# IvanIZ/BenchPush

Measured on AMD Instinct MI355X. Metric: env-steps/sec at N=4096 envs (ship-ice-v0), 1/2/4/8 MI355X, higher is better.
Workload: dtype f64

## Files before the change

benchpush_amd/csrc/bp_device.hpp:

```cpp
#pragma once
#include <hip/hip_runtime.h>
#include <stdint.h>

#include "../../include/benchpush_amd.h"

#define BP_KADJ 24
#define BP_ACAP 64

typedef double2 d2;

enum { BODY_DYNAMIC = 0, BODY_KINEMATIC = 1, BODY_STATIC = 2 };
__device__ __forceinline__ int kind_ctype(int k) { return k & 0xFF; }
__device__ __forceinline__ int kind_group(int k) { return (k >> 8) & 0xFF; }
__device__ __forceinline__ int kind_btype(int k) { return (k >> 16) & 3; }
enum { ARB_FIRST = 0, ARB_NORMAL = 1, ARB_IGNORE = 2, ARB_CACHED = 3 };
#define ARB_FREE_KEY 0xFFFFFFFFu

struct DevParams {
    double dt_sub;
    int steps, iterations, persistence, settle_steps;
    double damping_pow, bias_coef, slop, target_speed, max_yaw_rate, map_w, map_h, goal_y, m_to_pix;
    double beta, boundary_penalty, terminal_reward, local_w, local_h, vshift, obs_range;
    double goal_x, goal_reach, k_increment;
    int env_kind;
// ... 101 lines not shown
__device__ __forceinline__ double fclampd(double f, double lo, double hi) { return fmin(fmax(f, lo), hi); }

#define HW_PLANE_A(h) ((int)((h) & 31ull))
#define HW_PLANE_B(h) ((int)(((h) >> 5) & 31ull))
#define HW_VERT_A(h) ((int)(((h) >> 10) & 31ull))
#define HW_VERT_B(h) ((int)(((h) >> 15) & 31ull))
#define HW_NV_A(h) ((int)(((h) >> 20) & 31ull))
#define HW_NV_B(h) ((int)(((h) >> 25) & 31ull))
#define HW_HAS_A (1ull << 32)
#define HW_HAS_B (1ull << 33)
#define HW_PRIM_B (1ull << 34)
#define HW_BOTH (1ull << 35)
#define BP_SUPPORT_MARGIN 1e-10
#define BP_TIE_TOL 1e-9
#ifndef BP_QCAP
#define BP_QCAP 96
#endif

#define BP_CC_IDX_BITS 14
#define BP_EVCAP 32
#define BP_MBOX 16
#ifndef BP_NSLOT
#define BP_NSLOT 96
#endif
#define BP_PROFN 64
#define BP_SNAP_ROWS 9
#define BP_SNAP_COLS 12

struct LdsMap {
    unsigned sv, sw, sb, sp, ag, tf, q_dir, q_c, r_val, q_meta, q_aux, r_idx, pt_a, pt_thr, cc, cc_hw, res_smA, res_smB, res_iA, res_iB, res_jA, res_jB, mvs, owner, colmask, mvo, sbody, mv,
        slot_of, rf, ev_d, ev_key, ctl, snap, prof, total;
};
__host__ __device__ inline LdsMap bp_lds_map(const int nbcap, const int mvcap, const bool box, const bool prof)
{
    LdsMap m;
    unsigned p = 0;
    m.sv = p; p += 16u * (BP_NSLOT + 1);
    m.sw = p; p += 16u * (BP_NSLOT + 1);
    m.sb = p; p += 16u * (BP_NSLOT + 1);
    m.sp = p; p += 16u * (BP_NSLOT + 1);
    m.ag = p; p += 32u;
    m.tf = p;
    m.q_dir = p; p += 16u * BP_QCAP;
    m.q_c = p; p += 8u * BP_QCAP;
    m.r_val = p; p += 8u * BP_QCAP;
    m.q_meta = p; p += 4u * BP_QCAP;
    m.q_aux = p; p += 4u * BP_QCAP;
    m.r_idx = p; p += 4u * BP_QCAP;
    m.pt_a = p; p += 16u * 64;
    m.pt_thr = p; p += 16u * 64;
    m.cc = p; p += 8u * 64;
    m.cc_hw = p; p += 8u * 64;
    m.res_smA = p; p += 8u * 64;
    m.res_smB = p; p += 8u * 64;
    m.res_iA = p; p += 4u * 64;
    m.res_iB = p; p += 4u * 64;
    m.res_jA = p; p += 4u * 64;
    m.res_jB = p; p += 4u * 64;
    m.mvs = p; p += 4u * (unsigned)nbcap;
    m.owner = p; p += 2u * (BP_NSLOT + 2);
    m.colmask = p; p += 2u * (BP_NSLOT + 2);
    m.mvo = p; p += 4u * (BP_NSLOT + 2);
    m.sbody = p; p += 2u * (BP_NSLOT + 2);
    m.mv = p; p += 2u * (unsigned)mvcap;
    m.slot_of = p; p += (unsigned)nbcap;
    m.rf = p; p += 64u;
    p = (p + 15u) & ~15u;
    m.ev_d = p; if (box) p += 16u * 3 * BP_EVCAP;
    m.ev_key = p; if (box) p += 4u * BP_EVCAP;
    p = (p + 7u) & ~7u;
    m.ctl = p; if (box) p += 8u * 4;
    m.snap = p; if (box) p += 8u * BP_SNAP_ROWS * BP_SNAP_COLS;
    m.prof = p; if (prof) p += 8u * BP_PROFN;
    m.total = (p + 15u) & ~15u;
    return m;
}

struct BpImgHdr {
    unsigned stamp, stamp_start, costp, n_post, n_contact, n_first, ship_post, ship_contacts;
    int nmv, nslots, nlevels, yaw_violated, boundary_violated, wall_flag, cc_ok, cc_kmax, quiescent, pad_;
    unsigned long long prev_amask;
    double curr_dt, total_ke, total_imp, ecoef_e, ecoef;
};
#define BP_IMG_DROWS 20
#define BP_IMG_UROWS 11
#define BP_IMG_HDR 256
static_assert(sizeof(BpImgHdr) <= BP_IMG_HDR, "park image header");
__host__ __device__ inline unsigned bp_img_regs_off(const unsigned lds_bytes) { return (lds_bytes + 1023u) & ~1023u; }
__host__ __device__ inline unsigned bp_img_bytes(const unsigned lds_bytes) { return bp_img_regs_off(lds_bytes) + 512u * BP_IMG_DROWS + 256u * BP_IMG_UROWS + BP_IMG_HDR; }

#define SQ_MAXLEV 32
#define BP_DBL_MIN 2.2250738585072014e-308
#define BP_PI 3.14159265358979323846
#define BP_INF (__builtin_inf())

__device__ __forceinline__ void bp_sincos(double x, double &sn, double &cs)
{
    const double invpio2 = 6.36619772367581382433e-01;
    const double pio2_1 = 1.57079632673412561417e+00, pio2_1t = 6.07710050650619224932e-11;
    const double pio2_2 = 6.07710050630396597660e-11, pio2_2t = 2.02226624879595063154e-21;
    const double S1 = -1.66666666666666324348e-01, S2 = 8.33333333332248946124e-03, S3 = -1.98412698298579493134e-04,
                 S4 = 2.75573137070700676789e-06, S5 = -2.50507602534068634195e-08, S6 = 1.58969099521155010221e-10;
    const double C1 = 4.16666666666666019037e-02, C2 = -1.38888888888741095749e-03, C3 = 2.48015872894767294178e-05,
                 C4 = -2.75573143513906633035e-07, C5 = 2.08757232129817482790e-09, C6 = -1.13596475577881948265e-11;
    double fn = __builtin_rint(x * invpio2);
    double r = x - fn * pio2_1;
    double w = fn * pio2_1t;
    double y0 = r - w;
    const bool deep = __builtin_fabs(y0) < __builtin_fabs(x) * 7.62939453125e-06;
// ... 109 lines not shown
```

benchpush_amd/csrc/bp_physics.hpp:

```cpp
#pragma once
#include "bp_device.hpp"
#include <type_traits>

#ifdef BP_PROF
#define PROF_DECL unsigned long long _pt = __builtin_amdgcn_s_memtime();
#define PROF_ACC(slot) { unsigned long long _n = __builtin_amdgcn_s_memtime(); if (lane_id() == 0) L.prof[slot] += _n - _pt; _pt = _n; }
#define PROF_CNT(slot, v) { const unsigned long long _v = (unsigned long long)(v); if (lane_id() == 0) L.prof[slot] += _v; }
#define PROF_MAX(slot, v) { const unsigned long long _v = (unsigned long long)(v); if (lane_id() == 0 && _v > L.prof[slot]) L.prof[slot] = _v; }
#else
#define PROF_DECL
#define PROF_ACC(slot)
#define PROF_CNT(slot, v)
#define PROF_MAX(slot, v)
#endif


#define BP_UNLIKELY(x) __builtin_expect(!!(x), 0)
#define BP_UNLIKELY2(x) __builtin_expect(!!(x), 0)
#ifdef BP_DEBUG_PATHS
#define BP_DBGP(bit) ((P.dbg_paths & (bit)) != 0)
#define BP_TRACE_ON(D) ((D).dbg != nullptr)
#else
#define BP_DBGP(bit) false
#define BP_TRACE_ON(D) false
#endif
#ifndef BP_BOUND_GROUPS
#define BP_BOUND_GROUPS 3
#endif
#include "bp_contact.hpp"

struct EnvCtx {
    int nb;
    const int *nv;
    const d2 *lv, *ln;
    const double4 *mass;
    const double4 *prop;
    const int *kind;
    d2 *pxy, *rot, *wv, *wn, *pv;
    double *ang;
    double4 *bb, *fat;
    unsigned short *adj;
    unsigned char *adjn;
    unsigned long long *hint;
};

template <typename T> __device__ __forceinline__ T &gE(T *const base, const int idx) { return *(T *)((char *)base + (size_t)((unsigned)idx * (unsigned)sizeof(T))); }

struct LdsCtx {
    d2 *sv, *sw, *sb;
    d2 *ag;
    d2 *sp;
    unsigned char *slot_of;
    unsigned *mvs;
    unsigned short *owner;
    unsigned short *colmask;
    d2 *tf;
    unsigned short *mv;
    unsigned *mvo;
    unsigned short *sbody;
    unsigned char *rf;
    unsigned long long *res_smA, *res_smB;
    unsigned *res_iA, *res_iB, *res_jA, *res_jB;
    d2 *q_dir;
    double *q_c, *r_val;
    unsigned *q_meta, *q_aux, *r_idx;
    uint4 *pt_a;
    d2 *pt_thr;
    unsigned long long *cc, *cc_hw;
    d2 *mbox;
    unsigned *ev_key;
    d2 *ev_d;
    double *ctl;
    unsigned long long *snap;
#ifdef BP_PROF
    unsigned long long *prof;
#endif
};

struct SubState {
    unsigned stamp;
// ... 92 lines not shown
}

__device__ __forceinline__ void world_from_pose(const DevParams &P, const EnvCtx &E, int i, bool active, int q, double4 t,
                                                double4 &outbb)
{
    const int n = active ? gE(E.nv, i) : 0;
    const bool valid = active && (q < n);
    double vx = 0, vy = 0;
    if (valid) {
        const d2 lv = gE(E.lv, i * BP_MAXV + q), ln = gE(E.ln, i * BP_MAXV + q);
        const double c = t.x, s = t.y;
        vx = (c * lv.x + (-s) * lv.y) + t.z;
        vy = (s * lv.x + c * lv.y) + t.w;
        const double nx = c * ln.x + (-s) * ln.y;
        const double ny = s * ln.x + c * ln.y;
        gE(E.wv, i * BP_MAXV + q) = mk2(vx, vy);
        gE(E.wn, i * BP_MAXV + q) = mk2(nx, ny);
    }
    const double l = half_min(valid ? vx : BP_INF);
    const double r = half_max(valid ? vx : -BP_INF);
    const double bo = half_min(valid ? vy : BP_INF);
    const double tp = half_max(valid ? vy : -BP_INF);
    const double rad = gE(E.prop, i).x;
    outbb.x = l - rad; outbb.y = bo - rad; outbb.z = r + rad; outbb.w = tp + rad;
}

template <int VL>
__device__ __forceinline__ void support_queries(const EnvCtx &E, const LdsCtx &L, const int nq)
{
    const int lane = lane_id();
    const int l8 = lane & 7, g = lane >> 3;
    for (int base = 0; base < nq; base += 8) {
        const int k = base + g;
        const bool act = k < nq;
        const d2 dir = L.q_dir[act ? k : 0];
        const unsigned meta = L.q_meta[act ? k : 0];
        const int body = (int)(meta & 0xFFFFu), nv = (int)(meta >> 16);
        double best = BP_INF;
        int bi = 255;
#pragma unroll
        for (int t = 0; t < (VL + 7) / 8; t++) {
            const int q = l8 + 8 * t;
            const bool ok = act && (q < nv);
            const d2 v = gE(E.wv, body * BP_MAXV + (ok ? q : 0));
            const double d = vdot(dir, v);
            if (ok && d < best) { best = d; bi = q; }
        }
        const double m = oct_min_f64(best);
        const int mi = oct_min_i32((best == m) ? bi : 255);
        if (act && best == m && bi == mi) { L.r_val[k] = best; L.r_idx[k] = (unsigned)bi; }
    }
}

template <int KIND, bool DAMP = false>
__device__ __forceinline__ void substep(const DevParams &P, const EnvCtx &E, const LdsCtx &L, ArbReg &A, SubState &S,
                                        const double dt, const int ship_rules)
{
    const int lane = lane_id();
    constexpr int VL = (KIND == BP_ENV_BOX) ? 4 : (KIND == BP_ENV_MAZE) ? 8 : BP_MAXV;
    if (KIND == BP_ENV_BOX) { S.nev = 0; S.evmask = 0ull; }
    S.stamp += 1u;
    const unsigned now = S.stamp;
    const double prev_dt = S.curr_dt;
    S.curr_dt = dt;
    if (A.key != ARB_FREE_KEY && A.stamp == now - 1u) A.state = ARB_NORMAL;
    PROF_DECL
    PROF_CNT(16, S.nmv)

    for (int k0 = 0; k0 < S.nmv; k0 += 64) {
        const int k = k0 + lane;
        double rad = 0.0;
        double4 fatb; fatb.x = fatb.y = -BP_INF; fatb.z = fatb.w = BP_INF;
        if (k < S.nmv) {
            const int i = L.mv[k];
            const int sl = L.slot_of[i];
            d2 v = mk2(0.0, 0.0), w2 = mk2(0.0, 0.0), vb = mk2(0.0, 0.0);
            if (sl != 255) { v = L.sv[sl]; w2 = L.sw[sl]; vb = L.sb[sl]; }
            d2 p = gE(E.pxy, i);
            if (sl != 255) p = L.sp[sl];
            const double a = gE(E.ang, i);
            d2 r = gE(E.rot, i);
            const double4 ms = gE(E.mass, i);
            rad = gE(E.prop, i).x;
            fatb = gE(E.fat, i);
            L.rf[lane] = (unsigned char)gE(E.nv, i);
            p.x = p.x + (v.x + vb.x) * dt;
            p.y = p.y + (v.y + vb.y) * dt;
            const double a2 = a + (w2.x + w2.y) * dt;
            if (a2 != a) { double sn, cs; bp_sincos(a2, sn, cs); r = mk2(cs, sn); }
            gE(E.pxy, i) = p; gE(E.ang, i) = a2; gE(E.rot, i) = r;
            if (i == 0) { L.ag[0] = mk2(a2, 0.0); L.ag[1] = r; }
            if (sl != 255) { L.sb[sl] = mk2(0.0, 0.0); L.sw[sl].y = 0.0; L.sp[sl] = p; }
            double4 t;
            t.x = r.x; t.y = r.y;
            t.z = p.x - (ms.z * r.x - ms.w * r.y);
            t.w = p.y - (ms.z * r.y + ms.w * r.x);
            L.tf[2 * lane] = mk2(t.x, t.y);
            L.tf[2 * lane + 1] = mk2(t.z, t.w);
            L.mvs[i] = now;
        }
        const int cnt = min(64, S.nmv - k0);
        unsigned long long *bbk = L.res_smA;
        if (lane < cnt) { bbk[lane * 4 + 0] = ~0ull; bbk[lane * 4 + 1] = 0ull; bbk[lane * 4 + 2] = ~0ull; bbk[lane * 4 + 3] = 0ull; }
        lds_sync();
        PROF_ACC(33)
        for (int t0 = 0; t0 < cnt * VL; t0 += 64) {
            const int t = t0 + lane;
            const int kk = t / VL, q = t - kk * VL;
            if (kk < cnt) {
                const int i = L.mv[k0 + kk];
                if (q < (int)L.rf[kk]) {
                    const d2 t0_ = L.tf[2 * kk], t1_ = L.tf[2 * kk + 1];
// ... 122 lines not shown
        {
            const double dm = vdot(fnA, vAm), d0 = vdot(fnA, vA0), dp = vdot(fnA, vAp);
            if (evA && cnB == nB_h && cnB >= 2 && d0 + BP_SUPPORT_MARGIN <= dm && d0 + BP_SUPPORT_MARGIN <= dp && !BP_DBGP(4)) { sepAc = (d0 - cA) + 0.0; qryA = false; }
        }
        {
            const double dm = vdot(fnB, vBm), d0 = vdot(fnB, vB0), dp = vdot(fnB, vBp);
            if (evB && cnA == nA_h && cnA >= 2 && d0 + BP_SUPPORT_MARGIN <= dm && d0 + BP_SUPPORT_MARGIN <= dp && !BP_DBGP(4)) { sepBc = (d0 - cB) + 0.0; qryB = false; }
        }
        {
            const unsigned long long mqA = ballot(qryA), mqB = ballot(qryB);
            const int nqA = __popcll(mqA), nq1 = nqA + __popcll(mqB);
            PROF_CNT(37, nq1)
            if (BP_UNLIKELY(nq1)) {
                const int slA = popc_below(mqA, lane), slB = nqA + popc_below(mqB, lane);
                for (int q0 = 0; q0 < nq1; q0 += BP_QCAP) {
                    const bool inA = qryA && slA >= q0 && slA < q0 + BP_QCAP, inB = qryB && slB >= q0 && slB < q0 + BP_QCAP;
                    if (inA) { L.q_dir[slA - q0] = fnA; L.q_meta[slA - q0] = (unsigned)sb | ((unsigned)nB_h << 16); }
                    if (inB) { L.q_dir[slB - q0] = fnB; L.q_meta[slB - q0] = (unsigned)sa | ((unsigned)nA_h << 16); }
                    lds_sync();
                    support_queries<VL>(E, L, min(nq1 - q0, BP_QCAP));
                    lds_sync();
                    if (inA) { sepAc = (L.r_val[slA - q0] - cA) + 0.0; jAc = (int)L.r_idx[slA - q0]; }
                    if (inB) { sepBc = (L.r_val[slB - q0] - cB) + 0.0; jBc = (int)L.r_idx[slB - q0]; }
                    lds_sync();
                }
            }
        }
        if (valid && (sepAc > rsum || sepBc > rsum)) {
            valid = false;
            if (hw & HW_BOTH) {
                const unsigned long long nh = (hw & ~(HW_BOTH | HW_PRIM_B)) | ((sepAc > rsum) ? 0ull : HW_PRIM_B);
                gE(E.hint, i * BP_KADJ + s) = nh;
                if (base == 0) L.cc_hw[lane] = nh;
            }
        }
        const unsigned long long cm = ballot(valid);
        PROF_ACC(28)
        PROF_CNT(18, __popcll(cm))
        if (cm == 0) continue;
        PROF_CNT(25, 1)
        const int nc = __popcll(cm);
        const int myr = popc_below(cm, lane);
        const int nA_l = valid ? nA_h : 0, nB_l = valid ? nB_h : 0;
        if (valid) {
            uint4 pa;
            pa.x = (unsigned)sa | ((unsigned)sb << 16);
            pa.y = (unsigned)nA_l | (evA ? 0x80u : 0u) | ((unsigned)nB_l << 8) | ((unsigned)hA << 16) | ((unsigned)jAc << 24);
            pa.z = (unsigned)sb | ((unsigned)sa << 16);
            pa.w = (unsigned)nB_l | (evB ? 0x80u : 0u) | ((unsigned)nA_l << 8) | ((unsigned)hB << 16) | ((unsigned)jBc << 24);
            L.pt_a[myr] = pa;
            L.pt_thr[myr] = mk2(sepAc, sepBc);
            L.res_smA[myr] = evA ? f64_key(sepAc) : 0ull; L.res_iA[myr] = evA ? ((unsigned)hA << 8) | (unsigned)jAc : 0xFFFFFFFFu;
            L.res_smB[myr] = evB ? f64_key(sepBc) : 0ull; L.res_iB[myr] = evB ? ((unsigned)hB << 8) | (unsigned)jBc : 0xFFFFFFFFu;
        }
        lds_sync();
        {
            int nq = 0, g0 = 0;
            const uint2 *const pts = (const uint2 *)L.pt_a;
            const double *const pts_thr = (const double *)L.pt_thr;
            auto round_addr = [&](const uint2 e, int &pbody, int &qbody, int &np, int &nqv, int &hX, bool &evX, int &jc, int &jm, int &jp) {
                pbody = (int)(e.x & 0xFFFFu); qbody = (int)(e.x >> 16);
                np = (int)(e.y & 0x7Fu); evX = (e.y & 0x80u) != 0; nqv = (int)((e.y >> 8) & 0xFFu);
                hX = (int)((e.y >> 16) & 0xFFu); jc = (int)(e.y >> 24);
                jm = (jc == 0) ? max(nqv, 1) - 1 : jc - 1; jp = (jc + 1 >= nqv) ? 0 : jc + 1;
            };
            int rr_start = nc;
            {
                constexpr int GW = (BP_BOUND_GROUPS == 3 && KIND != BP_ENV_BOX) ? BP_MAXV + 1 : 32, IPR = 64 / GW;
                static_assert(GW >= BP_MAXV && IPR * GW <= 64, "a lane group holds every plane of a side");
                const int g = lane / GW, f = lane - g * GW;
                const int ipr = BP_DBGP(16) ? 1 : IPR;
                bool fits = !BP_DBGP(2);
                for (int r0 = 0; r0 < nc && fits; r0 += ipr) {
                    const bool on0 = g < ipr && 2 * r0 + g < 2 * nc, on1 = g < ipr && 2 * r0 + ipr + g < 2 * nc;
                    const int ta = on0 ? 2 * r0 + g : 2 * r0, tb = on1 ? 2 * r0 + ipr + g : 2 * r0;
                    const uint2 e0 = pts[ta], e1 = pts[tb];
                    const double th0 = pts_thr[ta], th1 = pts_thr[tb];
                    int pb0, qb0, np0, nqv0, hX0, jc0, jm0, jp0, pb1, qb1, np1, nqv1, hX1, jc1, jm1, jp1; bool ev0, ev1;
                    round_addr(e0, pb0, qb0, np0, nqv0, hX0, ev0, jc0, jm0, jp0);
                    round_addr(e1, pb1, qb1, np1, nqv1, hX1, ev1, jc1, jm1, jp1);
                    const int fc0 = (f < np0) ? f : 0, fc1 = (f < np1) ? f : 0;
                    const d2 fn0 = gE(E.wn, pb0 * BP_MAXV + fc0), fp0 = gE(E.wv, pb0 * BP_MAXV + fc0), vb0 = gE(E.wv, qb0 * BP_MAXV + jc0), vm0 = gE(E.wv, qb0 * BP_MAXV + jm0), vp0 = gE(E.wv, qb0 * BP_MAXV + jp0);
                    const d2 fn1 = gE(E.wn, pb1 * BP_MAXV + fc1), fp1 = gE(E.wv, pb1 * BP_MAXV + fc1), vb1 = gE(E.wv, qb1 * BP_MAXV + jc1), vm1 = gE(E.wv, qb1 * BP_MAXV + jm1), vp1 = gE(E.wv, qb1 * BP_MAXV + jp1);
                    {
                        const bool pv = on0 && (f < np0) && !(ev0 && f == hX0);
                        const double c = vdot(fn0, fp0);
                        const double bound = (fmin(vdot(fn0, vb0), fmin(vdot(fn0, vm0), vdot(fn0, vp0))) - c) + 0.0;
                        const bool surv = pv && (!ev0 || bound >= th0);
                        const unsigned long long sm = ballot(surv);
                        const int sl = nq + popc_below(sm, lane);
                        if (surv && sl < BP_QCAP) {
                            L.q_dir[sl] = fn0; L.q_meta[sl] = (unsigned)qb0 | ((unsigned)nqv0 << 16);
                            L.q_aux[sl] = (unsigned)(ta >> 1) | ((unsigned)(ta & 1) << 8) | ((unsigned)f << 16);
                            L.q_c[sl] = c;
                        }
                        nq += __popcll(sm);
                    }
                    {
                        const bool pv = on1 && (f < np1) && !(ev1 && f == hX1);
                        const double c = vdot(fn1, fp1);
                        const double bound = (fmin(vdot(fn1, vb1), fmin(vdot(fn1, vm1), vdot(fn1, vp1))) - c) + 0.0;
                        const bool surv = pv && (!ev1 || bound >= th1);
                        const unsigned long long sm = ballot(surv);
                        const int sl = nq + popc_below(sm, lane);
                        if (surv && sl < BP_QCAP) {
                            L.q_dir[sl] = fn1; L.q_meta[sl] = (unsigned)qb1 | ((unsigned)nqv1 << 16);
// ... 20 lines not shown
                        const int sl = s0 + lane;
                        if (sl < nq) {
                            const unsigned aux = L.q_aux[sl];
                            const int r = (int)(aux & 0xFFu);
                            const double sp = (L.r_val[sl] - L.q_c[sl]) + 0.0;
                            const unsigned long long key = f64_key(sp);
                            L.q_c[sl] = __builtin_bit_cast(double, key);
                            atomicMax((aux & 0x100u) ? &L.res_smB[r] : &L.res_smA[r], key);
                        }
                    }
                    lds_sync();
                    if (valid && myr >= g0 && myr < rr) {
                        if (evA && f64_key(sepAc) != L.res_smA[myr]) L.res_iA[myr] = 0xFFFFFFFFu;
                        if (evB && f64_key(sepBc) != L.res_smB[myr]) L.res_iB[myr] = 0xFFFFFFFFu;
                    }
                    lds_sync();
                    for (int s0 = 0; s0 < nq; s0 += 64) {
                        const int sl = s0 + lane;
                        if (sl < nq) {
                            const unsigned aux = L.q_aux[sl];
                            const int r = (int)(aux & 0xFFu);
                            const unsigned long long key = __builtin_bit_cast(unsigned long long, L.q_c[sl]);
                            if (key == ((aux & 0x100u) ? L.res_smB[r] : L.res_smA[r])) atomicMin((aux & 0x100u) ? &L.res_iB[r] : &L.res_iA[r], ((aux >> 16) << 8) | L.r_idx[sl]);
                        }
                    }
                    lds_sync();
                    nq = 0; g0 = rr;
                    PROF_ACC(30)
                }
                if (rr == nc) break;
                const uint2 e = pts[2 * rr + side];
                const double th = pts_thr[2 * rr + side];
                int pbody, qbody, np, nqv, hX, jc, jm, jp; bool evX;
                round_addr(e, pbody, qbody, np, nqv, hX, evX, jc, jm, jp);
                const bool pv = (f < np) && !(evX && f == hX);
                const int fc = (f < np) ? f : 0;
                const d2 fn = gE(E.wn, pbody * BP_MAXV + fc), fp = gE(E.wv, pbody * BP_MAXV + fc);
                const d2 vb = gE(E.wv, qbody * BP_MAXV + jc), vm = gE(E.wv, qbody * BP_MAXV + jm), vp = gE(E.wv, qbody * BP_MAXV + jp);
                const double c = vdot(fn, fp);
                const double bound = (fmin(vdot(fn, vb), fmin(vdot(fn, vm), vdot(fn, vp))) - c) + 0.0;
                const bool surv = pv && (!evX || bound >= th);
                const unsigned long long sm = ballot(surv);
                if (surv) {
                    const int sl = nq + popc_below(sm, lane);
                    L.q_dir[sl] = fn; L.q_meta[sl] = (unsigned)qbody | ((unsigned)nqv << 16);
                    L.q_aux[sl] = (unsigned)rr | ((unsigned)side << 8) | ((unsigned)f << 16);
                    L.q_c[sl] = c;
                }
                nq += __popcll(sm);
                lds_sync();
            }
        }
        PROF_ACC(3)
        Manifold M;
        M.count = 0; M.h0 = M.h1 = 0; M.n = mk2(0, 0);
        M.p1_0 = M.p2_0 = M.p1_1 = M.p2_1 = mk2(0, 0);
        bool touching = false;
        int src = 2;
        d2 n = mk2(0, 0);
        int iA = 0, iB = 0, jA = 0, jB = 0;
        int i1A = 0, i1B = 0;
        bool needA = false, needB = false;
        const int nA = nA_l, nB = nB_l;
        const d2 *Av = E.wv + sa * BP_MAXV, *Bv = E.wv + sb * BP_MAXV;
        const int oA = sa * BP_MAXV, oB = sb * BP_MAXV;
        if (valid) {
            const double sA = key_f64(L.res_smA[myr]), sB = key_f64(L.res_smB[myr]);
            const unsigned wA = L.res_iA[myr], wB = L.res_iB[myr];
            iA = (int)(wA >> 8); iB = (int)(wB >> 8); jA = (int)(wA & 0xFFu); jB = (int)(wB & 0xFFu);
            const bool useA = (sA >= sB);
            const double smax = useA ? sA : sB;
            touching = true;
            const int iA0 = (iA == 0) ? nA - 1 : iA - 1, iB0 = (iB == 0) ? nB - 1 : iB - 1;
            const d2 nAi = gE(E.wn, oA + iA), nBi = gE(E.wn, oB + iB);
            const d2 aA = gE(E.wv, oA + iA0), bA = gE(E.wv, oA + iA), qA = gE(E.wv, oB + jA);
            const d2 aB = gE(E.wv, oB + iB0), bB = gE(E.wv, oB + iB), qB = gE(E.wv, oA + jB);
            const int iA0m = (iA0 == 0) ? nA - 1 : iA0 - 1, iAp = (iA + 1 >= nA) ? 0 : iA + 1;
            const int iB0m = (iB0 == 0) ? nB - 1 : iB0 - 1, iBp = (iB + 1 >= nB) ? 0 : iB + 1;
            const d2 oA0 = gE(E.wv, oA + iA0m), oA1 = gE(E.wv, oA + iAp), oB0 = gE(E.wv, oB + iB0m), oB1 = gE(E.wv, oB + iBp);
            if (smax > rsum) touching = false;
            else if (smax <= 0.0) { n = useA ? nAi : vneg(nBi); src = useA ? 0 : 1; }
            else {
                const d2 eA = vsub(bA, aA);
                const double uA = vdot(vsub(qA, aA), eA), eeA = vdot(eA, eA);
                const bool spanA = !(uA < 0.0) && !(uA > eeA);
                const d2 eB = vsub(bB, aB);
                const double uB = vdot(vsub(qB, aB), eB), eeB = vdot(eB, eB);
                const bool spanB = !(uB < 0.0) && !(uB > eeB);
                auto tie_partner = [&](const d2 aP, const d2 eP, const double eeP, const d2 nP, const d2 *Qv, const int nQ, const int j, const d2 q0, const double u) -> bool {
                    const int jn = (u < 0.0) ? ((j == 0) ? nQ - 1 : j - 1) : ((j + 1 >= nQ) ? 0 : j + 1);
                    const d2 q1 = Qv[jn];
                    const double u1 = vdot(vsub(q1, aP), eP);
                    return !(u1 < 0.0) && !(u1 > eeP) && (vdot(nP, q1) - vdot(nP, q0) <= BP_TIE_TOL);
                };
                if (useA) {
                    if (spanA) { n = nAi; src = 0; }
                    else if (sB > 0.0 && spanB) { n = vneg(nBi); src = 1; }
                    else if (tie_partner(aA, eA, eeA, nAi, Bv, nB, jA, qA, uA)) { n = nAi; src = 0; }
                    else if (sB > 0.0 && tie_partner(aB, eB, eeB, nBi, Av, nA, jB, qB, uB)) { n = vneg(nBi); src = 1; }
                    else {
                        const d2 pp = vsub(qA, (uA < 0.0) ? aA : bA);
                        const double dl = vlen(pp);
                        if (dl > rsum) touching = false;
                        n = vmul(pp, 1.0 / (dl + BP_DBL_MIN));
                    }
                } else {
// ... 61 lines not shown
            }
            const double r1 = radA, r2 = radB;
            const double d_e1_a = vcross(e1a, n), d_e1_b = vcross(e1b, n);
            const double d_e2_a = vcross(e2a, n), d_e2_b = vcross(e2b, n);
            const double e1_denom = 1.0 / (d_e1_b - d_e1_a + BP_DBL_MIN);
            const double e2_denom = 1.0 / (d_e2_b - d_e2_a + BP_DBL_MIN);
            M.n = n;
            {
                const d2 p1 = vadd(vmul(n, r1), vlerp(e1a, e1b, clamp01((d_e2_b - d_e1_a) * e1_denom)));
                const d2 p2 = vadd(vmul(n, -r2), vlerp(e2a, e2b, clamp01((d_e1_a - d_e2_a) * e2_denom)));
                const double dist = vdot(vsub(p2, p1), n);
                if (dist <= 0.0) { M.p1_0 = p1; M.p2_0 = p2; M.h0 = ((unsigned)e1ia << 8) | (unsigned)e2ib; M.count = 1; }
            }
            {
                const d2 p1 = vadd(vmul(n, r1), vlerp(e1a, e1b, clamp01((d_e2_a - d_e1_a) * e1_denom)));
                const d2 p2 = vadd(vmul(n, -r2), vlerp(e2a, e2b, clamp01((d_e1_b - d_e2_a) * e2_denom)));
                const double dist = vdot(vsub(p2, p1), n);
                if (dist <= 0.0) {
                    const unsigned h = ((unsigned)e1ib << 8) | (unsigned)e2ia;
                    if (M.count == 0) { M.p1_0 = p1; M.p2_0 = p2; M.h0 = h; M.count = 1; }
                    else { M.p1_1 = p1; M.p2_1 = p2; M.h1 = h; M.count = 2; }
                }
            }
        }
        PROF_ACC(10)
        if (KIND == BP_ENV_BOX) {
            const bool ev = valid && M.count > 0 && (flagonly || (kind_ctype(gE(E.kind, sa)) == 2 && kind_ctype(gE(E.kind, sb)) == 3));
            const unsigned long long em = ballot(ev);
            if (em) {
                const int pos = S.nev + popc_below(em, lane);
                if (ev && pos < BP_EVCAP) {
                    L.ev_key[pos] = ((unsigned)sa << 16) | (unsigned)sb;
                    L.ev_d[pos * 3 + 0] = M.n;
                    L.ev_d[pos * 3 + 1] = vsub(M.p1_0, gE(E.pxy, sa));
                    L.ev_d[pos * 3 + 2] = vsub(M.p2_0, gE(E.pxy, sb));
                }
                S.nev += __popcll(em);
                if (S.nev > BP_EVCAP) { S.nev = BP_EVCAP; S.err |= BP_ERR_ARB_OVERFLOW; }
            }
        }
        if (ballot(valid && flagonly && M.count > 0)) S.wall_flag = 1;
        const unsigned long long dm = ballot(valid && !flagonly && M.count > 0);
        const int drank = popc_below(dm, lane);
        const int ndel = __popcll(dm);
        lds_sync();
        for (int dbase = 0; dbase < ndel; dbase += BP_MBOX) {
            const bool mine = valid && !flagonly && M.count > 0 && drank >= dbase && drank < dbase + BP_MBOX;
            if (mine) {
                d2 *mb = L.mbox + (drank - dbase) * 6;
                mb[0] = M.n; mb[1] = M.p1_0; mb[2] = M.p2_0; mb[3] = M.p1_1; mb[4] = M.p2_1;
                mb[5] = mk2(__hiloint2double((int)M.h0, M.count), __hiloint2double((int)M.h1, 0));
            }
            lds_sync();
            int my_mb = -1;
            bool fresh = false;
            unsigned long long m = dm;
            int dr = 0;
            const unsigned keyv = ((unsigned)sa << 16) | (unsigned)sb;
            while (m) {
                const int l = __ffsll((long long)m) - 1;
                m &= m - 1;
                if (dr >= dbase && dr < dbase + BP_MBOX) {
                    const unsigned key = (unsigned)__builtin_amdgcn_readlane((int)keyv, l);
                    const bool own = (A.key == key);
                    if (BP_UNLIKELY2(!ballot(own))) {
                        const unsigned long long om = ballot(A.key == ARB_FREE_KEY);
                        if (!om) S.err |= BP_ERR_ARB_OVERFLOW;
                        else {
                            const int owner = __ffsll((long long)om) - 1;
                            const int s1 = slot_get(L, S, E.pxy, (int)(key >> 16)), s2 = slot_get(L, S, E.pxy, (int)(key & 0xFFFFu));
                            if (lane == owner) { my_mb = dr - dbase; fresh = true; A.key = key; A.slotA = s1; A.slotB = s2; }
                        }
                    } else if (own) my_mb = dr - dbase;
                }
                dr++;
            }
            if (my_mb >= 0) {
                const d2 *mb = L.mbox + my_mb * 6;
                const d2 mn_ = mb[0], mp10 = mb[1], mp20 = mb[2], mp11 = mb[3], mp21 = mb[4], mh = mb[5];
                const d2 pa = L.sp[A.slotA], pbp = L.sp[A.slotB];
                const unsigned mh0 = (unsigned)__double2hiint(mh.x), mh1 = (unsigned)__double2hiint(mh.y);
                const int mcount = __double2loint(mh.x);
                if (BP_UNLIKELY2(fresh)) {
                    const int usa = (int)(A.key >> 16), usb = (int)(A.key & 0xFFFFu);
                    arbiter_adopt(A, gE(E.mass, usa), gE(E.mass, usb), gE(E.prop, usa), gE(E.prop, usb));
                }
                arbiter_update(A, mn_, mp10, mp20, mp11, mp21, mh0, mh1, mcount, pa, pbp, now);
            }
            lds_sync();
        }
    }
    S.cc_ok = 1;
    PROF_ACC(4)
    if (KIND == BP_ENV_BOX) {
        if (S.nev == 0 && S.nmv == P.nkin && ballot(A.key != ARB_FREE_KEY) == 0) {
            if (S.prev_amask != 0ull) { S.prev_amask = 0ull; S.nlevels = 0; }
            S.costp += 16u;
            S.ship_post = 0u; S.ship_contacts = 0u;
            S.quiescent = 0;
            PROF_ACC(9)
            return;
        }
    }
    if (A.key != ARB_FREE_KEY && A.stamp == now - 1u) {
        const int a = (int)(A.key >> 16), b = (int)(A.key & 0xFFFFu);
        if (L.mvs[a] != now && L.mvs[b] != now) A.stamp = now;
    }
    if (KIND == BP_ENV_BOX && S.nev > 0) {
        __syncthreads();
        unsigned last = 0u;
        for (int e = 0; e < S.nev; e++) {
            unsigned best = 0xFFFFFFFFu; int bi = 0;
            for (int q = 0; q < S.nev; q++) { const unsigned k = L.ev_key[q]; if ((e == 0 || k > last) && k < best) { best = k; bi = q; } }
            last = best;
            const int a = (int)(best >> 16), b = (int)(best & 0xFFFFu);
            const d2 n = L.ev_d[bi * 3 + 0], r1 = L.ev_d[bi * 3 + 1], r2 = L.ev_d[bi * 3 + 2];
            const int sl = L.slot_of[a];
            const d2 v = (sl != 255) ? L.sv[sl] : mk2(0.0, 0.0);
            const double f = 2 * (v.x * n.x + v.y * n.y);
            const d2 refl = mk2(v.x - n.x * f, v.y - n.y * f);
            const d2 nv = mk2(refl.x * 0.5, refl.y * 0.5);
            const d2 pa = gE(E.pxy, a), pb = gE(E.pxy, b);
            const double depth = vdot(vsub(vadd(pb, r2), vadd(pa, r1)), n);
            const d2 pn = mk2(pa.x + n.x * depth, pa.y + n.y * depth);
            const bool robot = a < P.nkin;
            if (robot) S.robot_hit = depth < 0;
            __syncthreads();
            if (robot) {
                if (lane < P.nkin) { gE(E.pxy, lane) = pn; L.sp[lane] = pn; L.sv[lane] = nv; }
                if (pn.x != pa.x || pn.y != pa.y) S.evmask |= 1ull;
            } else {
                if (lane == 0) { gE(E.pxy, a) = pn; if (sl != 255) { L.sv[sl] = nv; L.sp[sl] = pn; } }
                if (pn.x != pa.x || pn.y != pa.y) S.evmask |= 1ull << a;
            }
            __syncthreads();
        }
    }
    arbiter_filter(A, now, P.persistence);
    const bool active = (A.key != ARB_FREE_KEY) && (A.stamp == now);
    const unsigned long long amask = ballot(active);
    const int ba = (int)(A.key >> 16), bbi = (int)(A.key & 0xFFFFu);
// ... 379 lines not shown
```

Baseline: 293,100.

## Split contact manifold construction across lane pairs using DPP mate exchanges

For non-box environments, each candidate contact pair's manifold is now built by two adjacent lanes, one per shape side. The lanes swap separation, feature indices and clip points through DPP quad-permute moves, where previously one lane did the whole manifold serially. Up to 32 pairs are handled per round, which adds parallelism and shortens per-lane dependency chains. The cost is more ballots, extra LDS layout coupling (res_smB and res_iB must sit right after their A arrays), and more code complexity. Arbiter update logic is factored into a shared helper.

Measured after the change: 299,300, median of 6. +2.1%, better.

```diff
diff --git a/benchpush_amd/csrc/bp_device.hpp b/benchpush_amd/csrc/bp_device.hpp
--- a/benchpush_amd/csrc/bp_device.hpp
+++ b/benchpush_amd/csrc/bp_device.hpp
@@ -177,9 +177,9 @@
     m.cc = p; p += 8u * 64;
     m.cc_hw = p; p += 8u * 64;
     m.res_smA = p; p += 8u * 64;
-    m.res_smB = p; p += 8u * 64;
+    m.res_smB = m.res_smA + 8u * 64; p += 8u * 64;
     m.res_iA = p; p += 4u * 64;
-    m.res_iB = p; p += 4u * 64;
+    m.res_iB = m.res_iA + 4u * 64; p += 4u * 64;
     m.res_jA = p; p += 4u * 64;
     m.res_jB = p; p += 4u * 64;
     m.mvs = p; p += 4u * (unsigned)nbcap;
diff --git a/benchpush_amd/csrc/bp_physics.hpp b/benchpush_amd/csrc/bp_physics.hpp
--- a/benchpush_amd/csrc/bp_physics.hpp
+++ b/benchpush_amd/csrc/bp_physics.hpp
@@ -7,11 +7,15 @@
 #define PROF_ACC(slot) { unsigned long long _n = __builtin_amdgcn_s_memtime(); if (lane_id() == 0) L.prof[slot] += _n - _pt; _pt = _n; }
 #define PROF_CNT(slot, v) { const unsigned long long _v = (unsigned long long)(v); if (lane_id() == 0) L.prof[slot] += _v; }
 #define PROF_MAX(slot, v) { const unsigned long long _v = (unsigned long long)(v); if (lane_id() == 0 && _v > L.prof[slot]) L.prof[slot] = _v; }
+#define PROF_PARAM , unsigned long long &_pt
+#define PROF_ARG , _pt
 #else
 #define PROF_DECL
 #define PROF_ACC(slot)
 #define PROF_CNT(slot, v)
 #define PROF_MAX(slot, v)
+#define PROF_PARAM
+#define PROF_ARG
 #endif
 
 
@@ -26,6 +30,9 @@
 #endif
 #ifndef BP_BOUND_GROUPS
 #define BP_BOUND_GROUPS 3
+#endif
+#ifndef BP_MANIFOLD_LANES
+#define BP_MANIFOLD_LANES 2
 #endif
 #include "bp_contact.hpp"
 
@@ -224,12 +231,204 @@
     }
 }
 
+__device__ __forceinline__ void arbiters_take(const EnvCtx &E, const LdsCtx &L, ArbReg &A, SubState &S, const unsigned long long dm, const int dbase,
+                                              const unsigned keyv, const unsigned now)
+{
+    const int lane = lane_id();
+    int my_mb = -1;
+    bool fresh = false;
+    unsigned long long m = dm;
+    int dr = 0;
+    while (m) {
+        const int l = __ffsll((long long)m) - 1;
+        m &= m - 1;
+        if (dr >= dbase && dr < dbase + BP_MBOX) {
+            const unsigned key = (unsigned)__builtin_amdgcn_readlane((int)keyv, l);
+            const bool own = (A.key == key);
+            if (BP_UNLIKELY2(!ballot(own))) {
+                const unsigned long long om = ballot(A.key == ARB_FREE_KEY);
+                if (!om) S.err |= BP_ERR_ARB_OVERFLOW;
+                else {
+                    const int owner = __ffsll((long long)om) - 1;
+                    const int s1 = slot_get(L, S, E.pxy, (int)(key >> 16)), s2 = slot_get(L, S, E.pxy, (int)(key & 0xFFFFu));
+                    if (lane == owner) { my_mb = dr - dbase; fresh = true; A.key = key; A.slotA = s1; A.slotB = s2; }
+                }
+            } else if (own) my_mb = dr - dbase;
+        }
+        dr++;
+    }
+    if (my_mb >= 0) {
+        const d2 *mb = L.mbox + my_mb * 6;
+        const d2 mn_ = mb[0], mp10 = mb[1], mp20 = mb[2], mp11 = mb[3], mp21 = mb[4], mh = mb[5];
+        const d2 pa = L.sp[A.slotA], pbp = L.sp[A.slotB];
+        const unsigned mh0 = (unsigned)__double2hiint(mh.x), mh1 = (unsigned)__double2hiint(mh.y);
+        const int mcount = __double2loint(mh.x);
+        if (BP_UNLIKELY2(fresh)) {
+            const int usa = (int)(A.key >> 16), usb = (int)(A.key & 0xFFFFu);
+            arbiter_adopt(A, gE(E.mass, usa), gE(E.mass, usb), gE(E.prop, usa), gE(E.prop, usb));
+        }
+        arbiter_update(A, mn_, mp10, mp20, mp11, mp21, mh0, mh1, mcount, pa, pbp, now);
+    }
+}
+
+__device__ __forceinline__ int mate_i32(const int v) { return __builtin_amdgcn_update_dpp(v, v, 0xB1, 0xF, 0xF, false); }
+__device__ __forceinline__ double mate_f64(const double v) { return dpp_mov_f64<0xB1>(v); }
+__device__ __forceinline__ d2 mate_d2(const d2 v) { return mk2(mate_f64(v.x), mate_f64(v.y)); }
+
+template <int VL>
+__device__ __forceinline__ void manifold_lanes(const DevParams &P, const EnvCtx &E, const LdsCtx &L, ArbReg &A, SubState &S, const int nc, const bool first_round,
+                                               const unsigned now PROF_PARAM)
+{
+    const int lane = lane_id();
+    const int sd = lane & 1;
+    const int ppt = BP_DBGP(64) ? 1 : 32;
+    const uint2 *const pts = (const uint2 *)L.pt_a;
+    const unsigned long long *const res_sm = L.res_smA;
+    const unsigned *const res_i = L.res_iA;
+    for (int r0 = 0; r0 < nc; r0 += ppt) {
+        PROF_CNT(50, 1)
+        const bool on = (lane >> 1) < ppt && r0 + (lane >> 1) < nc;
+        const int r = on ? r0 + (lane >> 1) : r0;
+        const uint2 e = pts[2 * r + sd];
+        const unsigned w = res_i[sd * 64 + r];
+        const double sO = key_f64(res_sm[sd * 64 + r]);
+        const unsigned cw = L.res_jA[r];
+        const int oO = (int)(e.x & 0xFFFFu) * BP_MAXV, oQ = (int)(e.x >> 16) * BP_MAXV;
+        const int nO = (int)(e.y & 0x7Fu), nQ = (int)((e.y >> 8) & 0xFFu);
+        const int iO = (int)(w >> 8), jO = (int)(w & 0xFFu);
+        const int iO0 = (iO == 0) ? nO - 1 : iO - 1;
+        const int iO0m = (iO0 == 0) ? nO - 1 : iO0 - 1, iOp = (iO + 1 >= nO) ? 0 : iO + 1;
+        const d2 nOi = gE(E.wn, oO + iO);
+        const d2 aO = gE(E.wv, oO + iO0), bO = gE(E.wv, oO + iO), qO = gE(E.wv, oQ + jO);
+        const d2 oO0 = gE(E.wv, oO + iO0m), oO1 = gE(E.wv, oO + iOp);
+        const double rO = gE(E.prop, (int)(e.x & 0xFFFFu)).x, rQ = gE(E.prop, (int)(e.x >> 16)).x;
+        const double rsum = sd ? rQ + rO : rO + rQ;
+        const double sQ = mate_f64(sO);
+        const unsigned wQ = (unsigned)mate_i32((int)w);
+        const int iQ = (int)(wQ >> 8), jQ = (int)(wQ & 0xFFu);
+        const bool prim = sd ? !(sQ >= sO) : (sO >= sQ);
+        const double smax = prim ? sO : sQ;
+        const bool far = smax > rsum, deep = smax <= 0.0;
+        const d2 eO = vsub(bO, aO);
+        const double uO = vdot(vsub(qO, aO), eO), eeO = vdot(eO, eO);
+        const bool spanO = !(uO < 0.0) && !(uO > eeO), posO = sO > 0.0;
+        const int xb = mate_i32((spanO ? 1 : 0) | (posO ? 2 : 0));
+        const bool spanQ = (xb & 1) != 0, posQ = (xb & 2) != 0;
+        const bool spanP = prim ? spanO : spanQ, spanS = prim ? spanQ : spanO, posS = prim ? posQ : posO;
+        const bool open = on && !far && !deep && !spanP && !(posS && spanS);
+        bool tieO = false;
+        if (open && (prim || posO)) {
+            const int jn = (uO < 0.0) ? ((jO == 0) ? nQ - 1 : jO - 1) : ((jO + 1 >= nQ) ? 0 : jO + 1);
+            const d2 q1 = gE(E.wv, oQ + jn);
+            const double u1 = vdot(vsub(q1, aO), eO);
+            tieO = !(u1 < 0.0) && !(u1 > eeO) && (vdot(nOi, q1) - vdot(nOi, qO) <= BP_TIE_TOL);
+        }
+        const bool tieQ = mate_i32(tieO ? 1 : 0) != 0;
+        const bool tieP = prim ? tieO : tieQ, tieS = prim ? tieQ : tieO;
+        const bool byP = deep || spanP || (!(posS && spanS) && tieP);
+        const bool byS = !byP && posS && (spanS || tieS);
+        const bool mine = prim ? byP : byS;
+        const bool vpair = !byP && !byS;
+        d2 nM = sd ? vneg(nOi) : nOi;
+        bool tO = true;
+        if (on && !far && vpair && prim) {
+            const d2 c = (uO < 0.0) ? aO : bO;
+            const d2 pp = sd ? vsub(c, qO) : vsub(qO, c);
+            const double dl = vlen(pp);
+            if (dl > rsum) tO = false;
+            nM = vmul(pp, 1.0 / (dl + BP_DBL_MIN));
+        }
+        const d2 nX = mate_d2(nM);
+        const bool tQ = mate_i32(tO ? 1 : 0) != 0;
+        const d2 n = (mine || (vpair && prim)) ? nM : nX;
+        const bool touching = on && !far && tO && tQ;
+        const d2 nO_ = sd ? vneg(n) : n;
+        PROF_CNT(51, (unsigned long long)__popcll(ballot(touching && sd == 0 && !vpair && mine)) | ((unsigned long long)__popcll(ballot(touching && sd == 1 && !vpair && mine)) << 32))
+        PROF_CNT(52, __popcll(ballot(touching && sd == 0 && vpair)))
+        int i1 = jQ;
+        bool need = touching && (mine || vpair);
+        if (touching && mine) {
+            const double c0 = vdot(aO, nO_), c1 = vdot(bO, nO_), o0 = vdot(oO0, nO_), o1 = vdot(oO1, nO_);
+            const double cm = (c0 > c1) ? c0 : c1, om = (o0 > o1) ? o0 : o1;
+            if ((nO == 2 || cm >= om + BP_SUPPORT_MARGIN) && !BP_DBGP(8)) { i1 = (c0 > c1) ? iO0 : (c1 > c0) ? iO : min(iO0, iO); need = false; }
+        }
+        if (on && sd == 0) {
+            const unsigned long long nh = hint_word(iO, iQ, jO, jQ, nO, nQ, prim, smax, rsum);
+            gE(E.hint, (int)(cw & ((1u << BP_CC_IDX_BITS) - 1u)) * BP_KADJ + (int)((cw >> BP_CC_IDX_BITS) & 31u)) = nh;
+            if (first_round) L.cc_hw[cw >> 20] = nh;
+        }
+        PROF_ACC(31)
+        {
+            const unsigned long long mq = ballot(need);
+            const int nq2 = __popcll(mq), sl = popc_below(mq, lane);
+            PROF_CNT(39, nq2)
+            PROF_CNT(53, (unsigned long long)__popcll(mq & 0x5555555555555555ull) | ((unsigned long long)__popcll(mq & 0xAAAAAAAAAAAAAAAAull) << 32))
+            for (int q0 = 0; q0 < nq2; q0 += BP_QCAP) {
+                const bool in = need && sl >= q0 && sl < q0 + BP_QCAP;
+                if (in) { L.q_dir[sl - q0] = vneg(nO_); L.q_meta[sl - q0] = (e.x & 0xFFFFu) | ((unsigned)nO << 16); }
+                lds_sync();
+                support_queries<VL>(E, L, min(nq2 - q0, BP_QCAP));
+                lds_sync();
+                if (in) i1 = (int)L.r_idx[sl - q0];
+                lds_sync();
+            }
+        }
+        PROF_ACC(32)
+        const int a0 = (i1 == 0) ? nO - 1 : i1 - 1, a2 = (i1 + 1 == nO) ? 0 : i1 + 1;
+        const d2 nO1 = gE(E.wn, oO + i1), nO2 = gE(E.wn, oO + a2), vO0 = gE(E.wv, oO + a0), vO1 = gE(E.wv, oO + i1), vO2 = gE(E.wv, oO + a2);
+        const bool fO = vdot(nO_, nO1) > vdot(nO_, nO2);
+        const d2 ea = fO ? vO0 : vO1, eb = fO ? vO1 : vO2;
+        const int eia = fO ? a0 : i1, eib = fO ? i1 : a2;
+        const double d_a = vcross(ea, n), d_b = vcross(eb, n);
+        const double denom = 1.0 / (d_b - d_a + BP_DBL_MIN);
+        const double dQ_a = mate_f64(d_a), dQ_b = mate_f64(d_b);
+        const d2 nr = vmul(n, sd ? -rO : rO);
+        const d2 pt0 = vadd(nr, vlerp(ea, eb, clamp01(((sd ? dQ_a : dQ_b) - d_a) * denom)));
+        const d2 pt1 = vadd(nr, vlerp(ea, eb, clamp01(((sd ? dQ_b : dQ_a) - d_a) * denom)));
+        const d2 ptX = mate_d2(sd ? pt0 : pt1);
+        const d2 p1 = sd ? ptX : pt0, p2 = sd ? pt1 : ptX;
+        const bool hit = touching && vdot(vsub(p2, p1), n) <= 0.0;
+        const int xh = mate_i32((hit ? 1 : 0) | (eib << 1));
+        const bool hitQ = (xh & 1) != 0;
+        const unsigned h = sd ? ((unsigned)(xh >> 1) << 8) | (unsigned)eia : ((unsigned)eia << 8) | (unsigned)(xh >> 1);
+        const bool any = hit || hitQ, two = hit && hitQ;
+        PROF_CNT(54, (unsigned long long)__popcll(ballot(sd == 0 && hit && !hitQ)) | ((unsigned long long)__popcll(ballot(sd == 0 && !hit && hitQ)) << 32))
+        PROF_CNT(55, __popcll(ballot(sd == 0 && two)))
+        PROF_ACC(10)
+        const bool flagonly = (cw & (1u << 19)) != 0;
+        if (ballot(any && flagonly)) S.wall_flag = 1;
+        const bool del = any && !flagonly;
+        const unsigned long long dm = ballot(del && sd == 0);
+        const int drank = popc_below(dm, lane & ~1);
+        const int ndel = __popcll(dm);
+        const unsigned keyv = (e.x << 16) | (e.x >> 16);
+        lds_sync();
+        for (int dbase = 0; dbase < ndel; dbase += BP_MBOX) {
+            if (del && drank >= dbase && drank < dbase + BP_MBOX) {
+                d2 *mb = L.mbox + (drank - dbase) * 6;
+                if (sd == 0) {
+                    mb[0] = n;
+                    if (hit) { mb[1] = p1; mb[2] = p2; mb[5].x = __hiloint2double((int)h, two ? 2 : 1); }
+                } else {
+                    if (!hitQ) { mb[1] = p1; mb[2] = p2; mb[5].x = __hiloint2double((int)h, 1); }
+                    mb[3] = two ? p1 : mk2(0, 0); mb[4] = two ? p2 : mk2(0, 0);
+                    mb[5].y = __hiloint2double(two ? (int)h : 0, 0);
+                }
+            }
+            lds_sync();
+            arbiters_take(E, L, A, S, dm, dbase, keyv, now);
+            lds_sync();
+        }
+    }
+}
+
 template <int KIND, bool DAMP = false>
 __device__ __forceinline__ void substep(const DevParams &P, const EnvCtx &E, const LdsCtx &L, ArbReg &A, SubState &S,
                                         const double dt, const int ship_rules)
 {
     const int lane = lane_id();
     constexpr int VL = (KIND == BP_ENV_BOX) ? 4 : (KIND == BP_ENV_MAZE) ? 8 : BP_MAXV;
+    constexpr bool ML2 = (BP_MANIFOLD_LANES == 2) && KIND != BP_ENV_BOX;
     if (KIND == BP_ENV_BOX) { S.nev = 0; S.evmask = 0ull; }
     S.stamp += 1u;
     const unsigned now = S.stamp;
@@ -458,6 +657,8 @@
             L.pt_thr[myr] = mk2(sepAc, sepBc);
             L.res_smA[myr] = evA ? f64_key(sepAc) : 0ull; L.res_iA[myr] = evA ? ((unsigned)hA << 8) | (unsigned)jAc : 0xFFFFFFFFu;
             L.res_smB[myr] = evB ? f64_key(sepBc) : 0ull; L.res_iB[myr] = evB ? ((unsigned)hB << 8) | (unsigned)jBc : 0xFFFFFFFFu;
+            static_assert(BP_CC_IDX_BITS + 5 <= 19 && BP_KADJ <= 32, "candidate lane's word: i | slot << BP_CC_IDX_BITS | flagonly << 19 | lane << 20");
+            if (ML2) L.res_jA[myr] = (unsigned)i | ((unsigned)s << BP_CC_IDX_BITS) | (flagonly ? 1u << 19 : 0u) | ((unsigned)lane << 20);
         }
         lds_sync();
         {
@@ -584,6 +785,7 @@
             }
         }
         PROF_ACC(3)
+        if (ML2 && !BP_DBGP(32)) { manifold_lanes<VL>(P, E, L, A, S, nc, base == 0, now PROF_ARG); continue; }
         Manifold M;
         M.count = 0; M.h0 = M.h1 = 0; M.n = mk2(0, 0);
         M.p1_0 = M.p2_0 = M.p1_1 = M.p2_1 = mk2(0, 0);
@@ -751,41 +953,7 @@
                 mb[5] = mk2(__hiloint2double((int)M.h0, M.count), __hiloint2double((int)M.h1, 0));
             }
             lds_sync();
-            int my_mb = -1;
-            bool fresh = false;
-            unsigned long long m = dm;
-            int dr = 0;
-            const unsigned keyv = ((unsigned)sa << 16) | (unsigned)sb;
-            while (m) {
-                const int l = __ffsll((long long)m) - 1;
-                m &= m - 1;
-                if (dr >= dbase && dr < dbase + BP_MBOX) {
-                    const unsigned key = (unsigned)__builtin_amdgcn_readlane((int)keyv, l);
-                    const bool own = (A.key == key);
-                    if (BP_UNLIKELY2(!ballot(own))) {
-                        const unsigned long long om = ballot(A.key == ARB_FREE_KEY);
-                        if (!om) S.err |= BP_ERR_ARB_OVERFLOW;
-                        else {
-                            const int owner = __ffsll((long long)om) - 1;
-                            const int s1 = slot_get(L, S, E.pxy, (int)(key >> 16)), s2 = slot_get(L, S, E.pxy, (int)(key & 0xFFFFu));
-                            if (lane == owner) { my_mb = dr - dbase; fresh = true; A.key = key; A.slotA = s1; A.slotB = s2; }
-                        }
-                    } else if (own) my_mb = dr - dbase;
-                }
-                dr++;
-            }
-            if (my_mb >= 0) {
-                const d2 *mb = L.mbox + my_mb * 6;
-                const d2 mn_ = mb[0], mp10 = mb[1], mp20 = mb[2], mp11 = mb[3], mp21 = mb[4], mh = mb[5];
-                const d2 pa = L.sp[A.slotA], pbp = L.sp[A.slotB];
-                const unsigned mh0 = (unsigned)__double2hiint(mh.x), mh1 = (unsigned)__double2hiint(mh.y);
-                const int mcount = __double2loint(mh.x);
-                if (BP_UNLIKELY2(fresh)) {
-                    const int usa = (int)(A.key >> 16), usb = (int)(A.key & 0xFFFFu);
-                    arbiter_adopt(A, gE(E.mass, usa), gE(E.mass, usb), gE(E.prop, usa), gE(E.prop, usb));
-                }
-                arbiter_update(A, mn_, mp10, mp20, mp11, mp21, mh0, mh1, mcount, pa, pbp, now);
-            }
+            arbiters_take(E, L, A, S, dm, dbase, ((unsigned)sa << 16) | (unsigned)sb, now);
             lds_sync();
         }
     }
```
